# Malfoy/Brisk

Hardware: AMD Instinct MI355X
Metric: distinct k-mers indexed/sec (k=63,m=21) (higher is better)
Workload: dtype u64; 1 GPU; 1x MI355X: 50M synthetic 150 bp reads per GPU, k=63 m=21 b=14, uint8 counts, 15x coverage; reads_per_gpu=50000000, total_reads=50000000, part_bits=24, genome_len=500000000, parallelism=single GPU

## Files before the change

### brisk_amd/csrc/brisk_capi.hip

```cpp
#include "brisk_kernels.hip"

#include <algorithm>
#include <atomic>
#include <cerrno>
#include <chrono>
#include <cmath>
#include <cstdio>
#include <cstdlib>
#include <cstring>
#include <mutex>
#include <new>
#include <string>
#include <thread>
#include <vector>

#include <fcntl.h>
#include <sys/stat.h>
#include <unistd.h>

#include "../../include/brisk_hip.h"

#if !defined(__HIP_DEVICE_COMPILE__) && defined(__x86_64__)
#include <immintrin.h>
#define BRISK_HOST_AVX2 1
#endif

namespace {

enum Slot { S_PACK, S_SYNTH, S_COUNT, S_SCAN, S_HIST, S_PSUM, S_TOUCHED, S_SCATTER, S_INSERT, S_QUERY, S_ENUM, S_LOOKUP, S_PROFILE, S_PROFILE_LONG, S_UPLOAD, S_NSLOTS };
const char* const kSlotNames[S_NSLOTS] = {"k_pack_ascii", "k_synth", "k_count_kmers", "k_scan", "k_part_hist", "k_psum", "k_touched_need",
                                          "k_scatter", "k_insert", "k_query", "k_enumerate", "k_lookup", "k_profile_reads", "k_profile_segments_and_fold",
                                          "host_upload_and_pack_wall"};
static_assert(S_NSLOTS <= BRISK_HIP_PROFILE_SLOTS, "brisk_hip_profile_read fills caller arrays of BRISK_HIP_PROFILE_SLOTS");

struct DevBuf {
    void* p = nullptr;
    size_t bytes = 0;
};

struct VmBuf {
    char* base = nullptr;
    size_t reserved = 0, mapped = 0, gran = 0;
    std::vector<hipMemGenericAllocationHandle_t> handles;
    std::vector<size_t> sizes;
};

constexpr size_t kPinBytes = 8192;
struct PendingEvent {
    int slot;
    hipEvent_t a, b;
};

struct Counters {
    struct Scan { unsigned long long n_rec; u32 overflow, pad; } scan;
    struct Touched { u32 n_touched, pad; unsigned long long need; } touched;
    struct Kmers { unsigned long long bound, n_long; } kmers;
    struct Work { u32 wc[2], n_left, pad; } work;
    struct Plan { u32 n_long, n_vr; } plan;
    u32 n_rerun, pad;
    unsigned long long kept;
    unsigned long long n_ovf;
    unsigned long long slice_sum;
    u32 upsert_done, pad2;
    struct Result { unsigned long long w[3]; } result;
    unsigned long long dbg_guard;
};
static_assert(sizeof(Counters::Scan) == sizeof(unsigned long long) + 2 * sizeof(u32) && sizeof(Counters::Touched) == 2 * sizeof(u32) + sizeof(unsigned long long), "ScanOut; k_touched, k_need");
static_assert(sizeof(Counters::Kmers) == 2 * sizeof(unsigned long long) && sizeof(Counters::Result) == 3 * sizeof(unsigned long long), "k_count_kmers: out[0..1]; k_checksum: out[0..2]");
static_assert(sizeof(Counters::Work) == 4 * sizeof(u32) && sizeof(Counters::Plan) == 2 * sizeof(u32), "32-bit counters throughout");
struct PinnedCounters : Counters {
    u32 n_huge;
    unsigned long long arena_used;
    unsigned long long n_rec_new;
    unsigned long long prof[3];
    unsigned long long answers;
};

}

struct brisk_hip_index {
    BriskParams P{};
    int device = 0;
    hipStream_t stream = nullptr;
    bool own_stream = false;
    std::string err;
    std::recursive_mutex call_mu;
    u64 n_parts = 0, n_buckets = 0;
    u64 max_batch_reads = 0;

    double* d_coef = nullptr;
// ... 442 lines not shown
                           (u32)HUGE_LIST_CAP);
        if (int lrc = launch_check(h, "k_need")) return lrc;
    }
    HIPCHK(h, fetch_ctr(h, &h->d_ctr->touched.need));
    HIPCHK(h, hipMemcpyAsync(&h->h_ctr->arena_used, h->ix.cursor, 8, hipMemcpyDeviceToHost, h->stream));
    h->h_ctr->n_huge = 0;
    if (huge_at) HIPCHK(h, hipMemcpyAsync(&h->h_ctr->n_huge, h->huge.p, 4, hipMemcpyDeviceToHost, h->stream));
    HIPCHK(h, hipStreamSynchronize(h->stream));
    h->arena_used_host = h->h_ctr->arena_used;
    const u32 n_huge = h->h_ctr->n_huge <= HUGE_LIST_CAP ? h->h_ctr->n_huge : 0u;
    h->ix.huge_at = n_huge ? huge_at : 0u;
    if ((rc = ensure_arena(h, h->h_ctr->touched.need + h->h_ctr->touched.need / 7 + (u64)h->insert_waves * ARENA_CHUNK))) return rc;
    {
        ProfScope ps(h, S_INSERT);
        HIPCHK(h, zero_ctr(h, &h->d_ctr->work));
        const u32 batches = (n_touched + WI_BATCH - 1) / WI_BATCH;
        static const u64 big_at = getenv("BRISK_INSERT_BIG_AT") ? (u64)atoll(getenv("BRISK_INSERT_BIG_AT")) : 64ull;
        const bool big = !bl && n_rec / n_touched > big_at;
        const RecSrc src{bl ? bl->bins : (u64*)h->parted.p, (const u64*)h->parted.p, bl ? bl->bin_cap : 0u};
        static const u32 wave_env = getenv("BRISK_INSERT_WAVES") ? (u32)atoi(getenv("BRISK_INSERT_WAVES")) : 0u;
        const bool sat = h->count_mode == BRISK_HIP_COUNTS_SATURATE;
        auto resident = [&](const void* fn, int cap_per_cu = 0) -> u32 {
            int per_cu = 0, cus = 0;
            if (hipOccupancyMaxActiveBlocksPerMultiprocessor(&per_cu, fn, 64, 0) != hipSuccess || per_cu <= 0) per_cu = 16;
            if (cap_per_cu && per_cu > cap_per_cu) per_cu = cap_per_cu;
            if (hipDeviceGetAttribute(&cus, hipDeviceAttributeMultiprocessorCount, h->device) != hipSuccess || cus <= 0) cus = 256;
            const u32 w = std::min<u32>((u32)per_cu * (u32)cus, h->insert_waves);
            static const bool dbg = getenv("BRISK_DEBUG_INSERT") != nullptr;
            if (dbg) fprintf(stderr, "[brisk_hip] k_insert: %d waves per CU x %d CUs resident, %u launched\n", per_cu, cus, wave_env ? std::min<u32>(w, wave_env) : w);
            return wave_env ? std::min<u32>(w, wave_env) : w;
        };
        static const bool generic_only = getenv("BRISK_INSERT_GENERIC") != nullptr;
        static const bool lean_off = getenv("BRISK_INSERT_LEAN") && !strcmp(getenv("BRISK_INSERT_LEAN"), "0");
        const bool lean = fresh && !generic_only && !lean_off && !h->entry_ids && !big && P.nw == 3 && P.kb == 49 && P.shift >= 1 && P.shift <= 4;
        if (lean) {
            if ((rc = ensure(h, h->left, (size_t)n_touched * 4))) return rc;
            static const bool dbg = getenv("BRISK_DEBUG_INSERT") != nullptr;
            if (dbg) {
                hipFuncAttributes fa{};
                int per_cu = 0;
                const void* fn = sat ? (const void*)k_insert_first<3, 49, 4, true> : (const void*)k_insert_first<3, 49, 4, false>;
                if (hipFuncGetAttributes(&fa, fn) == hipSuccess && hipOccupancyMaxActiveBlocksPerMultiprocessor(&per_cu, fn, 64, 0) == hipSuccess) {
                    fprintf(stderr, "[brisk_hip] k_insert_first: the occupancy query gives %d waves per CU, the kernel is built for at most %d\n", per_cu, 4 * WI_WAVES_PER_EU_FIRST_MAX);
                    per_cu = std::min(per_cu, 4 * WI_WAVES_PER_EU_FIRST_MAX);
                    fprintf(stderr, "[brisk_hip] k_insert_first: %d waves per CU, %d registers, %zu B of LDS, %zu B of scratch\n", per_cu, fa.numRegs, fa.sharedSizeBytes, fa.localSizeBytes);
                }
            }
        }
#define LAUNCH_INSERT_K(KERNEL, NW, KB, SH, SAT)                                                                                                                    \
    {                                                                                                                                                               \
        const dim3 grid(std::min<u32>(batches, resident((const void*)KERNEL<NW, KB, SH, SAT>)));                                                                  \
        hipLaunchKernelGGL((KERNEL<NW, KB, SH, SAT>), grid, dim3(64), 0, h->stream, P, src, (const PartDesc*)h->desc.p, n_touched, h->ix,                         \
                           h->d_ctr->work.wc);                                                                                                                      \
    }
#define LAUNCH_INSERT(NW, KB, SH)                                                                                                                                   \
    {                                                                                                                                                               \
        if (big && sat) LAUNCH_INSERT_K(k_insert_big, NW, KB, SH, true)                                                                                             \
        else if (big) LAUNCH_INSERT_K(k_insert_big, NW, KB, SH, false)                                                                                              \
        else if (sat) LAUNCH_INSERT_K(k_insert, NW, KB, SH, true)                                                                                                   \
        else LAUNCH_INSERT_K(k_insert, NW, KB, SH, false)                                                                                                           \
    }
#define LAUNCH_INSERT_FAST(NW, KB, SH)                                                                                                                              \
    {                                                                                                                                                               \
        if (big) LAUNCH_INSERT(NW, KB, SH)                                                                                                                          \
        else if (sat) LAUNCH_INSERT_K(k_insert_fast, NW, KB, SH, true)                                                                                              \
        else LAUNCH_INSERT_K(k_insert_fast, NW, KB, SH, false)                                                                                                      \
    }
#define LAUNCH_INSERT_LEAN_K(SH, SAT)                                                                                                                               \
    {                                                                                                                                                               \
        u32* const wc = h->d_ctr->work.wc;                                                                                                                          \
        u32* const n_left = &h->d_ctr->work.n_left;                                                                                                                 \
        const dim3 grid(std::min<u32>(batches, resident((const void*)k_insert_first<3, 49, SH, SAT>, 4 * WI_WAVES_PER_EU_FIRST_MAX)));                                                            \
        hipLaunchKernelGGL((k_insert_first<3, 49, SH, SAT>), grid, dim3(64), 0, h->stream, P, src, (const PartDesc*)h->desc.p, n_touched, h->ix, wc,                \
                           (u32*)h->left.p, n_left);                                                                                                                \
        if ((rc = launch_check(h, "k_insert_first"))) return rc;                                                                                                    \
        const dim3 grid2(std::min<u32>(batches, resident((const void*)k_insert_fast_listed<3, 49, SH, SAT>)));                                                     \
        hipLaunchKernelGGL((k_insert_fast_listed<3, 49, SH, SAT>), grid2, dim3(64), 0, h->stream, P, src, (const PartDesc*)h->desc.p, n_touched, h->ix, wc + 1,     \
                           (const u32*)h->left.p, (const u32*)n_left);                                                                                              \
    }
#define LAUNCH_INSERT_LEAN(SH)                                                                                                                                      \
    {                                                                                                                                                               \
        if (sat) LAUNCH_INSERT_LEAN_K(SH, true)                                                                                                                     \
        else LAUNCH_INSERT_LEAN_K(SH, false)                                                                                                                        \
    }
        if (lean && P.shift == 4) LAUNCH_INSERT_LEAN(4)
        else if (lean && P.shift == 3) LAUNCH_INSERT_LEAN(3)
        else if (lean && P.shift == 2) LAUNCH_INSERT_LEAN(2)
        else if (lean) LAUNCH_INSERT_LEAN(1)
        else if (!generic_only && P.nw == 3 && P.kb == 49 && P.shift == 4) LAUNCH_INSERT_FAST(3, 49, 4)
        else if (!generic_only && P.nw == 3 && P.kb == 49 && P.shift == 3) LAUNCH_INSERT_FAST(3, 49, 3)
        else if (!generic_only && P.nw == 3 && P.kb == 49 && P.shift == 2) LAUNCH_INSERT_FAST(3, 49, 2)
        else if (!generic_only && P.nw == 3 && P.kb == 49 && P.shift == 1) LAUNCH_INSERT_FAST(3, 49, 1)
        else if (!generic_only && P.nw == 2 && P.kb == 17 && P.shift == 4) LAUNCH_INSERT_FAST(2, 17, 4)
        else if (!generic_only && P.nw == 2 && P.kb == 17 && P.shift == 5) LAUNCH_INSERT_FAST(2, 17, 5)
        else if (!generic_only && P.nw == 2 && P.kb == 17 && P.shift == 6) LAUNCH_INSERT_FAST(2, 17, 6)
        else if (!generic_only && P.nw == 2 && P.kb == 20 && P.shift == 0) LAUNCH_INSERT_FAST(2, 20, 0)
        else LAUNCH_INSERT(0, 0, 0)
#undef LAUNCH_INSERT_LEAN
#undef LAUNCH_INSERT_LEAN_K
#undef LAUNCH_INSERT_FAST
#undef LAUNCH_INSERT
#undef LAUNCH_INSERT_K
        if ((rc = launch_check(h, big ? "k_insert_big" : "k_insert"))) return rc;
        if (h->trace) {
            std::string path = big ? "k_insert_big (in-place collapse for partitions of > 128 records)" : "k_insert";
            if (lean) {
                HIPCHK(h, fetch_ctr_sync(h, &h->d_ctr->work.n_left));
                const u32 n_left = h->h_ctr->work.n_left;
                path = "k_insert_first (fresh index): " + std::to_string(n_touched - n_huge - n_left) + " partitions lean, " + std::to_string(n_left) + " left over to k_insert";
            }
            fprintf(stderr, "[brisk_hip] path: insert of %llu records (%s layout, histogram %s) into %u partitions: %s, %u partitions to k_insert_huge\n", (unsigned long long)n_rec,
                    bl ? "binned" : "classic", have_hist ? "from the scan" : "counted here", n_touched, path.c_str(), n_huge);
        }
        if (n_huge) {
            if (sat) hipLaunchKernelGGL(k_insert_huge<true>, dim3(std::min<u32>(n_huge, 256u)), dim3(HG_THREADS), 0, h->stream, P, src, (const PartDesc*)h->desc.p,
                                        (const u32*)h->huge.p + 1, (const u32*)h->huge.p, h->ix);
            else hipLaunchKernelGGL(k_insert_huge<false>, dim3(std::min<u32>(n_huge, 256u)), dim3(HG_THREADS), 0, h->stream, P, src, (const PartDesc*)h->desc.p,
                                    (const u32*)h->huge.p + 1, (const u32*)h->huge.p, h->ix);
            if ((rc = launch_check(h, "k_insert_huge"))) return rc;
        }
    }
    h->nb_skmers += n_rec;
    h->dir_snapshot_valid = false;
    return BRISK_HIP_OK;
}

int launch_scan(brisk_hip_index* h, const u32* d_packed, const u64* d_starts, u64 n_items, const ScanOut& out, bool query_mode, bool plain,
                const ChunkCtl& cc, bool pos = false) {
    ProfScope ps(h, S_SCAN);
    if (plain && !pos) {
        BriskParams P = h->P;
        if (out.ret) {
            P.ext_bits -= P.cls_bits;
            P.cls_bits = 0;
        }
        hipLaunchKernelGGL(k_scan, dim3(nblocks(n_items, SCAN_BLOCK)), dim3(SCAN_BLOCK), 0, h->stream, P, d_packed, d_starts, n_items, h->d_coef,
                           out, query_mode ? 1 : 0);
    } else {
        const u32 bt = h->scan_waves * 64;
        const dim3 grid(nblocks(n_items, bt)), block(bt);
#define LAUNCH_SCAN2(NCH, MODE, KK, MM) \
    hipLaunchKernelGGL((k_scan2<NCH, MODE, KK, MM>), grid, block, h->scan_lds - scan_fixed_tabs(MM) * 8, h->stream, h->P, h->scfg, d_packed, d_starts, n_items, h->d_tabs, out, cc)
#define LAUNCH_SCAN2_MODES(NCH, KK, MM)                    \
    {                                                      \
        if (pos && cc.vreads) LAUNCH_SCAN2(NCH, 4, KK, MM);  \
// ... 3145 lines not shown
```

### brisk_amd/csrc/brisk_insert.hip

```cpp
#ifndef ARENA_CHUNK
#define ARENA_CHUNK 16384u
#endif
#ifndef INSERT_SLOTS
#define INSERT_SLOTS 8192u
#endif
#ifndef WI_WAVES_PER_EU
#define WI_WAVES_PER_EU 4
#endif
#ifdef BRISK_PHASE_PROF
__device__ unsigned long long g_phase[16];
#define PHASE_DECL unsigned long long ph_acc[12] = {0, 0, 0, 0, 0, 0, 0, 0, 0, 0, 0, 0}; unsigned long long ph_last = __builtin_amdgcn_s_memtime(); u32 dbg_cnt[16] = {0, 0, 0, 0, 0, 0, 0, 0, 0, 0, 0, 0, 0, 0, 0, 0};
#define PHASE(i) { const unsigned long long t_ = __builtin_amdgcn_s_memtime(); ph_acc[i] += t_ - ph_last; ph_last = t_; }
__device__ unsigned long long g_cnt[16];
#define PHASE_FLUSH { PHASE(10) if (threadIdx.x == 0) { _Pragma("unroll") for (int q_ = 0; q_ < 12; q_++) atomicAdd(&g_phase[q_], ph_acc[q_]); \
                                                         _Pragma("unroll") for (int q_ = 0; q_ < 16; q_++) atomicAdd(&g_cnt[q_], (unsigned long long)dbg_cnt[q_]); } }
#define CNT(i, v) dbg_cnt[i] += (v);
#else
#define PHASE_DECL
#define PHASE(i)
#define PHASE_FLUSH
#define CNT(i, v)
#endif
struct IndexDev {
    u64* keys;
// ... 196 lines not shown
                    hh[it] = (hh[it] + 1) & (tsize - 1);
                }
            }
        }
    }
}

template <u32 NW>
struct RecGeom {
    static constexpr u32 CW = 2 * NW + 1;
    static constexpr u32 RS = 2 * NW + 3;
    static constexpr u32 INFO = 2 * NW + 1;
};
template <u32 NW>
__device__ __forceinline__ void store_rec_words(u32* dst, const RecRegs& rr, u32 info) {
    const u64 c0 = rr.w0, c1 = NW > 1 ? rr.w1 : 0, c2 = NW > 2 ? rr.w2 : 0, c3 = NW > 3 ? rr.w3 : 0;
    const u64 s0 = c0 << 6, s1 = (c1 << 6) | (c0 >> 58), s2 = (c2 << 6) | (c1 >> 58), s3 = (c3 << 6) | (c2 >> 58);
    const u32 top = (u32)((NW == 1 ? c0 : NW == 2 ? c1 : NW == 3 ? c2 : c3) >> 58);
    dst[0] = (u32)s0;
    dst[1] = (u32)(s0 >> 32);
    if (NW > 1) { dst[2] = (u32)s1; dst[3] = (u32)(s1 >> 32); }
    if (NW > 2) { dst[4] = (u32)s2; dst[5] = (u32)(s2 >> 32); }
    if (NW > 3) { dst[6] = (u32)s3; dst[7] = (u32)(s3 >> 32); }
    dst[2 * NW] = top;
    dst[RecGeom<NW>::INFO] = info;
    dst[RecGeom<NW>::INFO + 1] = 0;
}
template <u32 NIMAX>
struct LaneInst {
    u64 klo[NIMAX], khi[NIMAX];
    u32 hh[NIMAX];
    u32 won;
};
template <u32 NI, u32 NW, u32 KB, u32 SHIFT, u32 NIMAX, bool FOLD, bool SAT>
__device__ __forceinline__ void expand_and_dedupe_words(u32 lane, u32 ninst, u32 tsize, const u32* s_rw, const uint8_t* s_irec, const uint8_t* s_imult,
                                                        const u32* s_rmult, u64* s_key, u32* s_tab, u32* dbg_rounds, LaneInst<NIMAX>& li) {
    constexpr u32 RS = RecGeom<NW>::RS, INFO = RecGeom<NW>::INFO, KBITS = 2 * KB + 6;
    static_assert(KBITS + SHIFT <= 128 && SHIFT <= 6, "entry key: [routing id low bits | compacted k-mer | idx']");
    static_assert(NI <= NIMAX, "instances per lane");
    u64 (&klo)[NIMAX] = li.klo;
    u64 (&khi)[NIMAX] = li.khi;
    u32 (&hh)[NIMAX] = li.hh;
    u32 mult[NI];
    u32 rix[NI];
    u32 won = 0;
#pragma unroll
    for (u32 it = 0; it < NI; it++) {
        const u32 i = it * 64 + lane;
        rix[it] = s_irec[i < ninst ? i : 0];
    }
#pragma unroll
    for (u32 it = 0; it < NI; it++) {
        const u32 i = it * 64 + lane;
        const u32* base = s_rw + rix[it] * RS;
        const u32 info = base[INFO];
        const u32 j = i < ninst ? i - (info & 0x3ffu) : 0;
        const u32 n = (info >> 10) & 0xffu;
        const u32 s = 2 * (n - 1 - j);
        const u32* wp = base + (s >> 5);
        const u32 sh = s & 31;
        const u32 w0 = wp[0], w1 = wp[1], w2 = wp[2], w3 = wp[3], w4 = wp[4];
        u32 k0 = __builtin_amdgcn_alignbit(w1, w0, sh), k1 = __builtin_amdgcn_alignbit(w2, w1, sh);
        u32 k2 = __builtin_amdgcn_alignbit(w3, w2, sh), k3 = __builtin_amdgcn_alignbit(w4, w3, sh);
        k0 = (k0 & ~0x3fu) | (((info >> 18) & 0xffu) + j);
        constexpr u32 m0 = KBITS >= 32 ? ~0u : (1u << KBITS) - 1, m1 = KBITS >= 64 ? ~0u : KBITS <= 32 ? 0u : (1u << (KBITS - 32)) - 1;
        constexpr u32 m2 = KBITS >= 96 ? ~0u : KBITS <= 64 ? 0u : (1u << (KBITS - 64)) - 1, m3 = KBITS >= 128 ? ~0u : KBITS <= 96 ? 0u : (1u << (KBITS - 96)) - 1;
        k0 &= m0; k1 &= m1; k2 &= m2; k3 &= m3;
        u64 lo = ((u64)k1 << 32) | k0, hi = ((u64)k3 << 32) | k2;
        if (SHIFT) {
            const u64 rl = (info >> 26) & ((1u << SHIFT) - 1);
            if (KBITS >= 64) hi |= rl << (KBITS - 64);
            else {
                lo |= rl << KBITS;
                if (KBITS + SHIFT > 64) hi |= rl >> (64 - KBITS);
            }
        }
        klo[it] = lo;
        khi[it] = hi;
        hh[it] = hash_key32(mk128(lo, hi)) & (tsize - 1);
        mult[it] = FOLD ? (u32)s_imult[i < ninst ? i : 0] << WI_CNT_SHIFT : count8<SAT>(s_rmult[rix[it]]) << WI_CNT_SHIFT;
        if (i < ninst) {
            s_key[2 * i] = lo;
            s_key[2 * i + 1] = hi;
        }
    }
    wave_sync();
    for (u32 w = 0; w * 64 < tsize; w++) s_tab[w * 64 + lane] = EMPTY_SLOT;
    wave_sync();
    u32 pending = 0;
#pragma unroll
    for (u32 it = 0; it < NI; it++)
        if (it * 64 + lane < ninst) pending |= 1u << it;
    while (__any(pending != 0)) {
        *dbg_rounds += NI;
        u32 old[NI];
#pragma unroll
        for (u32 it = 0; it < NI; it++) {
            old[it] = EMPTY_SLOT;
            if (pending >> it & 1) old[it] = atomicCAS(&s_tab[hh[it]], EMPTY_SLOT, (it * 64 + lane) | mult[it]);
        }
        u64 olo[NI], ohi[NI];
#pragma unroll
        for (u32 it = 0; it < NI; it++) {
            const u32 oi = old[it] == EMPTY_SLOT ? 0 : (old[it] & WI_IDX_MASK);
            olo[it] = s_key[2 * oi];
            ohi[it] = s_key[2 * oi + 1];
        }
#pragma unroll
        for (u32 it = 0; it < NI; it++) {
// ... 41 lines not shown
                break;
            }
            h = (h + 1) & (2 * WI_MAX_REC - 1);
        }
    }
    return dup;
}

#ifndef WI_FOLD_TRIPS
#define WI_FOLD_TRIPS 16u
#endif
struct FoldFrame {
    W4 u, m;
    u32 rid;
    u32 rng;
    u32 s;
};
template <u32 NW, u32 KB>
__device__ __forceinline__ FoldFrame fold_frame(const RecRegs& rr, u64 hdr, u32 n, bool valid, u32 frame_end, u32 lane) {
    FoldFrame f;
    const u32 idx0 = hdr_idx0(hdr), end = idx0 + n, top = frame_end - idx0 + KB - 1;
    const bool ok = valid && n > 0 && end <= frame_end && top <= 32 * NW;
    const u32 lo_bits = ok ? 2 * (frame_end - end) : 0, hi_bits = ok ? 2 * top : 0;
    f.m = w4_andn(w4_mask(hi_bits), w4_mask(lo_bits));
    f.u = w4_and(w4_shl(W4{rr.w0, NW > 1 ? rr.w1 : 0, NW > 2 ? rr.w2 : 0, NW > 3 ? rr.w3 : 0}, lo_bits), f.m);
    f.rid = hdr_bucket(hdr);
    f.rng = idx0 | (end << 8);
    f.s = ok ? (n << 6) | (63 - lane) : 0;
    return f;
}
__device__ __forceinline__ u64 readlane64(u64 v, u32 a) {
    return ((u64)(u32)__builtin_amdgcn_readlane((int)(v >> 32), (int)a) << 32) | (u32)__builtin_amdgcn_readlane((int)v, (int)a);
}
template <u32 NW>
__device__ __forceinline__ bool fold_records(const FoldFrame& f, u32 nrec, u32 lane, u32* lead, u32* off, u32* trips) {
    u32 sv = lane < nrec ? f.s : 0;
    bool folded = false;
    *lead = lane;
    *off = 0;
    for (u32 t = 0; t < WI_FOLD_TRIPS; t++) {
        const u32 smax = (u32)__builtin_amdgcn_readlane((int)wave_incl_max_scan(sv), 63);
        if (smax == 0) break;
        *trips += 1;
        const u32 a = 63 - (smax & 63);
        const u32 rid_a = (u32)__builtin_amdgcn_readlane((int)f.rid, (int)a), rng_a = (u32)__builtin_amdgcn_readlane((int)f.rng, (int)a);
        const u32 i0 = f.rng & 0xffu, e = f.rng >> 8, i0a = rng_a & 0xffu, ea = rng_a >> 8;
#ifdef BRISK_NO_RECORD_FOLD
        bool in = sv != 0 && rid_a == f.rid && i0a == i0 && ea == e;
#else
        bool in = sv != 0 && rid_a == f.rid && i0a <= i0 && e <= ea;
#endif
        bool same = (readlane64(f.u.w0, a) & f.m.w0) == f.u.w0;
        if (NW > 1) same = same & ((readlane64(f.u.w1, a) & f.m.w1) == f.u.w1);
        if (NW > 2) same = same & ((readlane64(f.u.w2, a) & f.m.w2) == f.u.w2);
        if (NW > 3) same = same & ((readlane64(f.u.w3, a) & f.m.w3) == f.u.w3);
        in = in && same;
        if (in) {
            sv = 0;
            if (lane != a) {
                folded = true;
                *lead = a;
                *off = i0 - i0a;
            }
        }
    }
    return folded;
}

template <u32 MAXI, u32 NW, u32 KB, u32 SHIFT, bool SAT, bool LISTED = false>
__device__ __forceinline__ void insert_body(const BriskParams& PP, const RecSrc& src, const PartDesc* __restrict__ desc, u32 n_touched_all, const IndexDev& ix,
                                            u32* __restrict__ work_counter, const u32* __restrict__ list = nullptr, const u32* __restrict__ n_list = nullptr) {
    const u32 n_touched = LISTED ? min(*n_list, n_touched_all) : n_touched_all;
    u64* const rec = src.rec;
    BriskParams P = PP;
    if (NW) {
        P.nw = NW;
        P.stride = NW + 1;
        P.kb = KB;
        P.shift = SHIFT;
    }
    constexpr u32 TABLE = 2 * MAXI, TS = TABLE / 64, NI = MAXI / 64;
    constexpr u32 KW = NW ? (2 * KB + 6 + SHIFT <= 64 ? 1u : 2u) : 0u;
    constexpr bool FOLD = NW >= 3 && MAXI == WI_MAX_INST;
    static_assert(MAXI % 256 == 0 && MAXI <= 1024, "chunk size: whole 32-bit words of record marks per lane, 10-bit instance index");
    constexpr u32 REC_U64 = WI_MAX_REC * 5 > MAXI / 2 ? WI_MAX_REC * 5 : MAXI / 2;
    static_assert(NW == 0 || (WI_MAX_REC * RecGeom<NW ? NW : 1>::RS + 4) * 4 <= REC_U64 * 8, "shifted record words must fit the record buffer");
    constexpr bool TAB_OVER_REC = NW && TABLE * 4 <= REC_U64 * 8;
    constexpr u32 OFF_REC = 16 * MAXI, OFF_TAB = TAB_OVER_REC ? OFF_REC : OFF_REC + 8 * REC_U64, OFF_RTAB = TAB_OVER_REC ? OFF_REC + 8 * REC_U64 : OFF_TAB + 4 * TABLE;
    constexpr u32 OFF_RMULT = OFF_RTAB + 4 * 2 * WI_MAX_REC, OFF_IREC = OFF_RMULT + 4 * WI_MAX_REC, OFF_PREF = OFF_IREC + MAXI;
    constexpr u32 LDS_BYTES = NW ? OFF_PREF : OFF_PREF + 4 * (WI_MAX_REC + 1) + 4;
    __shared__ __attribute__((aligned(16))) unsigned char s_mem[LDS_BYTES];
    u64* s_key = (u64*)s_mem;
    u32* s_idiff = (u32*)s_mem;
    u64* s_rec = (u64*)(s_mem + OFF_REC);
    u32* s_rw = (u32*)s_rec;
    u32* s_tab = (u32*)(s_mem + OFF_TAB);
    u32* s_list = (u32*)s_rec;
    u32* s_rtab = (u32*)(s_mem + OFF_RTAB);
// ... 392 lines not shown
__global__ void __launch_bounds__(64) __attribute__((amdgpu_waves_per_eu(WI_WAVES_PER_EU, 8))) k_insert(BriskParams P, RecSrc src, const PartDesc* __restrict__ desc,
                                               u32 n_touched, IndexDev ix, u32* __restrict__ work_counter) {
    insert_body<WI_MAX_INST, NW, KB, SHIFT, SAT>(P, src, desc, n_touched, ix, work_counter);
}
template <u32 NW, u32 KB, u32 SHIFT, bool SAT = false>
__global__ void __launch_bounds__(64) __attribute__((amdgpu_waves_per_eu(2, 8))) k_insert_big(BriskParams P, RecSrc src, const PartDesc* __restrict__ desc,
                                                                                         u32 n_touched, IndexDev ix, u32* __restrict__ work_counter) {
    insert_body<2 * WI_MAX_INST, NW, KB, SHIFT, SAT>(P, src, desc, n_touched, ix, work_counter);
}

#ifndef NI_LEAN
#define NI_LEAN 3
#endif
#ifndef WI_WAVES_PER_EU_FIRST
#define WI_WAVES_PER_EU_FIRST 6
#endif
#ifndef WI_WAVES_PER_EU_FIRST_MAX
#define WI_WAVES_PER_EU_FIRST_MAX 6
#endif
template <u32 NIL, u32 NW>
struct LeanLds {
    static constexpr u32 MAXI = 64 * NIL, TABLE = 512;
    static_assert((TABLE & (TABLE - 1)) == 0 && TABLE >= 2 * MAXI && TABLE <= 4 * MAXI, "probe table: a power of two, at most half full");
    static constexpr u32 REC_BYTES = (WI_MAX_REC * RecGeom<NW>::RS + 4) * 4;
    static constexpr u32 OFF_REC = 16 * MAXI;
    static constexpr u32 REGION = REC_BYTES > 4 * TABLE ? REC_BYTES : 4 * TABLE;
    static constexpr u32 OFF_IREC = OFF_REC + REGION, OFF_IMULT = OFF_IREC + MAXI, BYTES = OFF_IMULT + MAXI;
};
__device__ __forceinline__ unsigned long long first_lane64(unsigned long long v) {
    return ((unsigned long long)(u32)__builtin_amdgcn_readfirstlane((int)(v >> 32)) << 32) | (u32)__builtin_amdgcn_readfirstlane((int)v);
}
template <u32 NIL, u32 NW, u32 KB, u32 SHIFT, bool SAT>
__device__ __forceinline__ void insert_first_body(const BriskParams& P, const RecSrc& src, const PartDesc* __restrict__ desc, u32 n_touched, const IndexDev& ix,
                                                  u32* __restrict__ work_counter, u32* __restrict__ left_list, u32* __restrict__ n_left) {
    using L = LeanLds<NIL, NW>;
    constexpr u32 MAXI = L::MAXI, TABLE = L::TABLE, RS = RecGeom<NW>::RS, INFO = RecGeom<NW>::INFO, KBITS = 2 * KB + 6;
    constexpr u32 KW = KBITS + SHIFT <= 64 ? 1u : 2u;
    static_assert(NIL == 2 || NIL == 3, "instance slots per lane");
    static_assert(NW >= 3 && SHIFT < 5, "the folding k63 geometries: at most 16 buckets per partition");
    static_assert(L::BYTES <= 13 * 512, "LDS per wave: 24 waves must fit a CU's 160 KiB");
    static_assert(4 * MAXI <= 16 * MAXI, "the multiplicity steps lie over the keys");
    static_assert(MAXI + (MAXI >> 2) + 8 <= ARENA_CHUNK / 8, "grow_cap(MAXI) is a small request: the host's arena reserve covers the tail a refill strands");
    __shared__ __attribute__((aligned(16))) unsigned char s_mem[L::BYTES];
    u64* s_key = (u64*)s_mem;
    u32* s_idiff = (u32*)s_mem;
    u32* s_rw = (u32*)(s_mem + L::OFF_REC);
    u32* s_tab = (u32*)(s_mem + L::OFF_REC);
    uint8_t* s_irec = s_mem + L::OFF_IREC;
    uint8_t* s_imult = s_mem + L::OFF_IMULT;

    const u32 lane = threadIdx.x;
    PHASE_DECL
    unsigned long long acur = first_lane64(ix.slot_cur[blockIdx.x]), aend = first_lane64(ix.slot_end[blockIdx.x]), garbage = 0;
    const u32 frame_end = P.suff_reduc + P.w + 1;

    for (;;) {
        u32 t0 = 0;
        if (lane == 0) t0 = atomicAdd(work_counter, WI_BATCH);
        t0 = (u32)__builtin_amdgcn_readfirstlane((int)t0);
        if (t0 >= n_touched) break;
        const u32 t_end = min(t0 + WI_BATCH, n_touched);
        unsigned long long left_mask = 0;
        PartDesc d = desc[t0];
        RecRegs rr = load_part_recs(P, src, d.part, d.r_begin, d.r_begin, min(d.n_rec, (u32)WI_MAX_REC), lane);

        for (u32 t = t0; t < t_end; t++) {
            const u32 tn = t + 1;
            PartDesc dn{};
            if (tn < t_end) dn = desc[tn];
            asm volatile("" ::"v"(rr.w0), "v"(rr.w1), "v"(rr.w2), "v"(rr.w3), "v"(rr.w4));
            do {
                if (ix.huge_at && d.n_inst > ix.huge_at) break;
                CNT(0, 1)
                if (d.n_exist | d.cap | (u32)(d.n_rec > WI_MAX_REC)) {
                    left_mask |= 1ull << (t - t0);
                    break;
                }
                PHASE(0)
                const u32 part = d.part, nrec = d.n_rec;
                const u64 my_hdr = NW == 3 ? rr.w3 : rr.w4;
                const u32 raw_n = lane < nrec ? hdr_n(my_hdr) : 0;
                const u32 my_mult = (my_hdr & HDR_HAS_MULT) ? (u32)(my_hdr >> 48) & 0xffu : 1u;
                const u32 info_hi = (raw_n << 10) | (hdr_idx0(my_hdr) << 18) | ((hdr_bucket(my_hdr) & ((1u << SHIFT) - 1)) << 26);
                const FoldFrame ff = fold_frame<NW, KB>(rr, my_hdr, raw_n, lane < nrec, frame_end, lane);
                wave_sync();
                if (lane < nrec) store_rec_words<NW>(s_rw + lane * RS, rr, 0);
                u32 lead = lane, lead_off = 0, dbg_trips = 0;
                const bool dup = fold_records<NW>(ff, nrec, lane, &lead, &lead_off, &dbg_trips);
                const u32 my_n = (lane < nrec && !dup) ? raw_n : 0;
                const u32 x = wave_incl_scan(my_n, lane);
                const u32 ninst = (u32)__builtin_amdgcn_readlane((int)x, 63);
                if (ninst > MAXI) {
                    left_mask |= 1ull << (t - t0);
                    break;
                }
                PHASE(1)
                CNT(1, 1)
                const u32 m_first = (u32)__shfl(x - my_n, lead, 64) + lead_off;
                u32 tsize = 128;
                while (tsize < 4 * ninst && tsize < TABLE) tsize <<= 1;
                {
                    if (NIL == 2) ((uint16_t*)s_irec)[lane] = 0;
                    else {
#pragma unroll
                        for (u32 q = 0; q < NIL; q++) s_irec[q * 64 + lane] = 0;
                    }
#pragma unroll
                    for (u32 q = 0; q < NIL; q++) s_idiff[lane * NIL + q] = 0;
                    wave_sync();
                    if (my_n) s_irec[x - my_n] = (uint8_t)(lane + 1);
                    if (lane < nrec) {
                        atomicAdd(&s_idiff[m_first], my_mult);
                        if (m_first + raw_n < ninst) atomicAdd(&s_idiff[m_first + raw_n], 0u - my_mult);
                    }
                    wave_sync();
                    u32 mk[NIL], mv[NIL], run = 0, tot = 0;
                    if (NIL == 2) {
                        const u32 w = ((const uint16_t*)s_irec)[lane];
                        mk[0] = w & 0xff;
                        mk[1] = w >> 8;
                    } else {
// ... 5 lines not shown
                        run = op_max_u32(run, mk[q]);
                        tot += s_idiff[lane * NIL + q];
                        mv[q] = tot;
                    }
                    const u32 before = wave_incl_scan(tot, lane) - tot;
                    u32 carry = wave_prev_lane(wave_incl_max_scan(run));
#pragma unroll
                    for (u32 q = 0; q < NIL; q++) {
                        carry = op_max_u32(carry, mk[q]);
                        mk[q] = (carry - 1) & 0xff;
                        mv[q] = count8<SAT>(mv[q] + before) & 0xff;
                    }
                    if (NIL == 2) {
                        ((uint16_t*)s_irec)[lane] = (uint16_t)(mk[0] | (mk[1] << 8));
                        ((uint16_t*)s_imult)[lane] = (uint16_t)(mv[0] | (mv[1] << 8));
                    } else {
#pragma unroll
                        for (u32 q = 0; q < NIL; q++) {
                            s_irec[lane * NIL + q] = (uint8_t)mk[q];
                            s_imult[lane * NIL + q] = (uint8_t)mv[q];
                        }
                    }
                    if (lane < nrec) s_rw[lane * RS + INFO] = (x - my_n) | info_hi;
                }
                wave_sync();
                PHASE(2)
                CNT(3, (ninst + 63) / 64)
                CNT(4, ninst)
                CNT(5, nrec)
                CNT(11, dbg_trips)
                u32 dbg_r = 0;
                LaneInst<NIL> li;
                li.won = 0;
                if (ninst <= 64) expand_and_dedupe_words<1, NW, KB, SHIFT, NIL, true, SAT>(lane, ninst, tsize, s_rw, s_irec, s_imult, nullptr, s_key, s_tab, &dbg_r, li);
                else if (NIL == 2 || ninst <= 128) expand_and_dedupe_words<2, NW, KB, SHIFT, NIL, true, SAT>(lane, ninst, tsize, s_rw, s_irec, s_imult, nullptr, s_key, s_tab, &dbg_r, li);
                else expand_and_dedupe_words<NIL, NW, KB, SHIFT, NIL, true, SAT>(lane, ninst, tsize, s_rw, s_irec, s_imult, nullptr, s_key, s_tab, &dbg_r, li);
                wave_sync();
                CNT(8, dbg_r)
                PHASE(3)
                u32 n_new = 0, new_rank[NIL], new_word[NIL];
#pragma unroll
                for (u32 it = 0; it < NIL; it++) {
                    new_rank[it] = 0;
                    new_word[it] = 0;
                    if (it * 64 < ninst) {
                        const bool made = (li.won >> it) & 1;
                        if (made) new_word[it] = s_tab[li.hh[it]];
                        const unsigned long long bal = __ballot(made);
                        new_rank[it] = n_new + (u32)__popcll(bal & lanes_below(lane));
                        n_new += (u32)__popcll(bal);
                    }
                }
                wave_sync();
#ifndef INSERT_NO_EARLY_WAIT
                __builtin_amdgcn_s_waitcnt(0x0F70);
#endif
                PHASE(6)
                CNT(7, n_new)
                unsigned long long off = d.off;
                u32 cap = 0;
                if (n_new) {
                    const unsigned long long want = grow_cap(n_new);
                    if (acur + want > aend) {
                        garbage += aend - acur;
                        unsigned long long got = 0;
                        if (lane == 0) got = atomicAdd(ix.cursor, (unsigned long long)ARENA_CHUNK);
                        acur = first_lane64(got);
                        aend = acur + ARENA_CHUNK;
                    }
                    if (acur + want > ix.arena_cap) {
                        if (lane == 0) atomicOr(ix.err, 2u);
                        n_new = 0;
                    } else {
                        off = acur;
                        acur += want;
                        cap = (u32)want;
                    }
                }
                PHASE(7)
                u32 bm0 = 0;
#pragma unroll
                for (u32 it = 0; it < NIL; it++) {
                    if (it * 64 < ninst && ((li.won >> it) & 1) && n_new) {
                        const unsigned long long at = off + new_rank[it];
                        store_key<KW>(ix, at, li.klo[it], li.khi[it]);
                        ix.counts[at] = (uint8_t)count8<SAT>(new_word[it] >> WI_CNT_SHIFT);
                        const u32 bl = SHIFT ? ((u32)shr128(mk128(li.klo[it], li.khi[it]), KBITS).lo & ((1u << SHIFT) - 1)) : 0;
                        bm0 |= 1u << bl;
                    }
                }
                PHASE(8)
                bm0 = wave_or_all(bm0);
                if (lane == 0) {
                    ix.dir[part] = DirEnt{off, n_new, cap};
                    const u64 first = ((u64)part << SHIFT) >> P.ext_bits;
                    const u32 bits = bm0 << (first & 31);
                    if (bits && (!ix.bits_check || (ix.bucket_bits[first >> 5] & bits) != bits)) atomicOr(&ix.bucket_bits[first >> 5], bits);
                }
            } while (0);
            d = dn;
            if (tn < t_end) rr = load_part_recs(P, src, d.part, d.r_begin, d.r_begin, min(d.n_rec, (u32)WI_MAX_REC), lane);
            PHASE(9)
        }
        if (left_mask) {
            const u32 n = (u32)__popcll(left_mask);
            u32 at = 0;
            if (lane == 0) at = atomicAdd(n_left, n);
            at = (u32)__builtin_amdgcn_readfirstlane((int)at);
            if ((left_mask >> lane) & 1) left_list[at + (u32)__popcll(left_mask & lanes_below(lane))] = t0 + lane;
        }
    }
    PHASE_FLUSH
    if (lane == 0) {
        ix.slot_cur[blockIdx.x] = acur;
        ix.slot_end[blockIdx.x] = aend;
        if (garbage) atomicAdd(&ix.stats[3], garbage);
    }
}
template <u32 NW, u32 KB, u32 SHIFT, bool SAT = false, u32 NIL = NI_LEAN>
__global__ void __launch_bounds__(64) __attribute__((amdgpu_waves_per_eu(WI_WAVES_PER_EU_FIRST, WI_WAVES_PER_EU_FIRST_MAX))) k_insert_first(BriskParams P, RecSrc src, const PartDesc* __restrict__ desc,
                                                                                                          u32 n_touched, IndexDev ix, u32* __restrict__ work_counter,
                                                                                                          u32* __restrict__ left_list, u32* __restrict__ n_left) {
    insert_first_body<NIL, NW, KB, SHIFT, SAT>(P, src, desc, n_touched, ix, work_counter, left_list, n_left);
}

__global__ void __launch_bounds__(256) k_bucket_bits(BriskParams P, IndexDev ix, u32 n_parts) {
    const u32 kbits = 2 * P.kb + 6;
    for (u32 part = blockIdx.x; part < n_parts; part += gridDim.x) {
        const u32 cnt = ix.dir[part].cnt;
        const unsigned long long off = ix.dir[part].off;
        for (u32 e = threadIdx.x; e < cnt; e += blockDim.x) {
            const u128x key = load_key(ix, off + e);
            const u32 bucket = (part << P.shift) | ((u32)shr128(key, kbits).lo & ((1u << P.shift) - 1));
            const u32 bit = 1u << (bucket & 31);
            if (!(ix.bucket_bits[bucket >> 5] & bit)) atomicOr(&ix.bucket_bits[bucket >> 5], bit);
        }
    }
}

__global__ void __launch_bounds__(256) k_stats(const DirEnt* __restrict__ dir, u64 n_parts, const u32* __restrict__ bits, u64 n_words,
                                               unsigned long long* out ) {
    __shared__ unsigned long long s_a[4], s_b[4], s_c[4];
    unsigned long long a = 0, b = 0, c = 0;
    const u64 stride = (u64)gridDim.x * blockDim.x;
    for (u64 i = (u64)blockIdx.x * blockDim.x + threadIdx.x; i < n_parts; i += stride) {
        const u32 v = dir[i].cnt;
        a += v;
        c = v > c ? v : c;
    }
    for (u64 i = (u64)blockIdx.x * blockDim.x + threadIdx.x; i < n_words; i += stride) b += __popc(bits[i]);
    for (int o = 32; o > 0; o >>= 1) {
        a += __shfl_down(a, o, 64);
        b += __shfl_down(b, o, 64);
        const unsigned long long c2 = __shfl_down(c, o, 64);
        c = c2 > c ? c2 : c;
    }
// ... 211 lines not shown
```

Measured before the change: 29.61 billion k-mers/s.

## Skip LDS hash-table dedupe in lean insert when fold proves instances distinct

During record folding, the fresh-index lean insert path now checks whether any two records that share a minimizer core could produce overlapping k-mer instances. When none can, the partition is marked clean and its keys are expanded directly without the LDS hash-table dedupe, and ranks are assigned by instance index. This removes the hashing, table probing and extra wave syncs for most partitions. In exchange it adds a readlane comparison per fold trip, more register pressure in the hot kernel, a counter atomic, and a correctness risk if the distinctness test misses a duplicate.

```diff
diff --git a/brisk_amd/csrc/brisk_capi.hip b/brisk_amd/csrc/brisk_capi.hip
--- a/brisk_amd/csrc/brisk_capi.hip
+++ b/brisk_amd/csrc/brisk_capi.hip
@@ -55,7 +55,7 @@
     struct Scan { unsigned long long n_rec; u32 overflow, pad; } scan;
     struct Touched { u32 n_touched, pad; unsigned long long need; } touched;
     struct Kmers { unsigned long long bound, n_long; } kmers;
-    struct Work { u32 wc[2], n_left, pad; } work;
+    struct Work { u32 wc[2], n_left, n_clean; } work;
     struct Plan { u32 n_long, n_vr; } plan;
     u32 n_rerun, pad;
     unsigned long long kept;
@@ -564,6 +564,7 @@
         };
         static const bool generic_only = getenv("BRISK_INSERT_GENERIC") != nullptr;
         static const bool lean_off = getenv("BRISK_INSERT_LEAN") && !strcmp(getenv("BRISK_INSERT_LEAN"), "0");
+        static const bool clean_off = getenv("BRISK_INSERT_CLEAN") && !strcmp(getenv("BRISK_INSERT_CLEAN"), "0");
         const bool lean = fresh && !generic_only && !lean_off && !h->entry_ids && !big && P.nw == 3 && P.kb == 49 && P.shift >= 1 && P.shift <= 4;
         if (lean) {
             if ((rc = ensure(h, h->left, (size_t)n_touched * 4))) return rc;
@@ -602,9 +603,10 @@
     {                                                                                                                                                               \
         u32* const wc = h->d_ctr->work.wc;                                                                                                                          \
         u32* const n_left = &h->d_ctr->work.n_left;                                                                                                                 \
+        u32* const n_clean = clean_off ? nullptr : &h->d_ctr->work.n_clean;                                                                                         \
         const dim3 grid(std::min<u32>(batches, resident((const void*)k_insert_first<3, 49, SH, SAT>, 4 * WI_WAVES_PER_EU_FIRST_MAX)));                                                            \
         hipLaunchKernelGGL((k_insert_first<3, 49, SH, SAT>), grid, dim3(64), 0, h->stream, P, src, (const PartDesc*)h->desc.p, n_touched, h->ix, wc,                \
-                           (u32*)h->left.p, n_left);                                                                                                                \
+                           (u32*)h->left.p, n_left, n_clean);                                                                                                       \
         if ((rc = launch_check(h, "k_insert_first"))) return rc;                                                                                                    \
         const dim3 grid2(std::min<u32>(batches, resident((const void*)k_insert_fast_listed<3, 49, SH, SAT>)));                                                     \
         hipLaunchKernelGGL((k_insert_fast_listed<3, 49, SH, SAT>), grid2, dim3(64), 0, h->stream, P, src, (const PartDesc*)h->desc.p, n_touched, h->ix, wc + 1,     \
@@ -635,14 +637,15 @@
 #undef LAUNCH_INSERT_K
         if ((rc = launch_check(h, big ? "k_insert_big" : "k_insert"))) return rc;
         if (h->trace) {
-            std::string path = big ? "k_insert_big (in-place collapse for partitions of > 128 records)" : "k_insert";
+            std::string path = big ? "k_insert_big (in-place collapse for partitions of > 128 records)" : "k_insert", tail;
             if (lean) {
-                HIPCHK(h, fetch_ctr_sync(h, &h->d_ctr->work.n_left));
+                HIPCHK(h, fetch_ctr_sync(h, &h->d_ctr->work));
                 const u32 n_left = h->h_ctr->work.n_left;
                 path = "k_insert_first (fresh index): " + std::to_string(n_touched - n_huge - n_left) + " partitions lean, " + std::to_string(n_left) + " left over to k_insert";
+                tail = " (" + std::to_string(h->h_ctr->work.n_clean) + " table-free)";
             }
-            fprintf(stderr, "[brisk_hip] path: insert of %llu records (%s layout, histogram %s) into %u partitions: %s, %u partitions to k_insert_huge\n", (unsigned long long)n_rec,
-                    bl ? "binned" : "classic", have_hist ? "from the scan" : "counted here", n_touched, path.c_str(), n_huge);
+            fprintf(stderr, "[brisk_hip] path: insert of %llu records (%s layout, histogram %s) into %u partitions: %s, %u partitions to k_insert_huge%s\n", (unsigned long long)n_rec,
+                    bl ? "binned" : "classic", have_hist ? "from the scan" : "counted here", n_touched, path.c_str(), n_huge, tail.c_str());
         }
         if (n_huge) {
             if (sat) hipLaunchKernelGGL(k_insert_huge<true>, dim3(std::min<u32>(n_huge, 256u)), dim3(HG_THREADS), 0, h->stream, P, src, (const PartDesc*)h->desc.p,
diff --git a/brisk_amd/csrc/brisk_insert.hip b/brisk_amd/csrc/brisk_insert.hip
--- a/brisk_amd/csrc/brisk_insert.hip
+++ b/brisk_amd/csrc/brisk_insert.hip
@@ -252,10 +252,56 @@
     u32 hh[NIMAX];
     u32 won;
 };
+template <u32 NW, u32 KB, u32 SHIFT>
+__device__ __forceinline__ void cut_key(const u32* base, u32 i, u32 ninst, u64* lo_out, u64* hi_out) {
+    constexpr u32 INFO = RecGeom<NW>::INFO, KBITS = 2 * KB + 6;
+    const u32 info = base[INFO];
+    const u32 j = i < ninst ? i - (info & 0x3ffu) : 0;
+    const u32 n = (info >> 10) & 0xffu;
+    const u32 s = 2 * (n - 1 - j);
+    const u32* wp = base + (s >> 5);
+    const u32 sh = s & 31;
+    const u32 w0 = wp[0], w1 = wp[1], w2 = wp[2], w3 = wp[3], w4 = wp[4];
+    u32 k0 = __builtin_amdgcn_alignbit(w1, w0, sh), k1 = __builtin_amdgcn_alignbit(w2, w1, sh);
+    u32 k2 = __builtin_amdgcn_alignbit(w3, w2, sh), k3 = __builtin_amdgcn_alignbit(w4, w3, sh);
+    k0 = (k0 & ~0x3fu) | (((info >> 18) & 0xffu) + j);
+    constexpr u32 m0 = KBITS >= 32 ? ~0u : (1u << KBITS) - 1, m1 = KBITS >= 64 ? ~0u : KBITS <= 32 ? 0u : (1u << (KBITS - 32)) - 1;
+    constexpr u32 m2 = KBITS >= 96 ? ~0u : KBITS <= 64 ? 0u : (1u << (KBITS - 64)) - 1, m3 = KBITS >= 128 ? ~0u : KBITS <= 96 ? 0u : (1u << (KBITS - 96)) - 1;
+    k0 &= m0; k1 &= m1; k2 &= m2; k3 &= m3;
+    u64 lo = ((u64)k1 << 32) | k0, hi = ((u64)k3 << 32) | k2;
+    if (SHIFT) {
+        const u64 rl = (info >> 26) & ((1u << SHIFT) - 1);
+        if (KBITS >= 64) hi |= rl << (KBITS - 64);
+        else {
+            lo |= rl << KBITS;
+            if (KBITS + SHIFT > 64) hi |= rl >> (64 - KBITS);
+        }
+    }
+    *lo_out = lo;
+    *hi_out = hi;
+}
+template <u32 NI, u32 NW, u32 KB, u32 SHIFT, u32 NIMAX>
+__device__ __forceinline__ void expand_words_distinct(u32 lane, u32 ninst, const u32* s_rw, const uint8_t* s_irec, LaneInst<NIMAX>& li) {
+    static_assert(NI <= NIMAX, "instances per lane");
+    u32 rix[NI];
+    u32 won = 0;
+#pragma unroll
+    for (u32 it = 0; it < NI; it++) {
+        const u32 i = it * 64 + lane;
+        rix[it] = s_irec[i < ninst ? i : 0];
+    }
+#pragma unroll
+    for (u32 it = 0; it < NI; it++) {
+        const u32 i = it * 64 + lane;
+        cut_key<NW, KB, SHIFT>(s_rw + rix[it] * RecGeom<NW>::RS, i, ninst, &li.klo[it], &li.khi[it]);
+        if (i < ninst) won |= 1u << it;
+    }
+    li.won = won;
+}
 template <u32 NI, u32 NW, u32 KB, u32 SHIFT, u32 NIMAX, bool FOLD, bool SAT>
 __device__ __forceinline__ void expand_and_dedupe_words(u32 lane, u32 ninst, u32 tsize, const u32* s_rw, const uint8_t* s_irec, const uint8_t* s_imult,
                                                         const u32* s_rmult, u64* s_key, u32* s_tab, u32* dbg_rounds, LaneInst<NIMAX>& li) {
-    constexpr u32 RS = RecGeom<NW>::RS, INFO = RecGeom<NW>::INFO, KBITS = 2 * KB + 6;
+    constexpr u32 RS = RecGeom<NW>::RS, KBITS = 2 * KB + 6;
     static_assert(KBITS + SHIFT <= 128 && SHIFT <= 6, "entry key: [routing id low bits | compacted k-mer | idx']");
     static_assert(NI <= NIMAX, "instances per lane");
     u64 (&klo)[NIMAX] = li.klo;
@@ -272,29 +318,8 @@
 #pragma unroll
     for (u32 it = 0; it < NI; it++) {
         const u32 i = it * 64 + lane;
-        const u32* base = s_rw + rix[it] * RS;
-        const u32 info = base[INFO];
-        const u32 j = i < ninst ? i - (info & 0x3ffu) : 0;
-        const u32 n = (info >> 10) & 0xffu;
-        const u32 s = 2 * (n - 1 - j);
-        const u32* wp = base + (s >> 5);
-        const u32 sh = s & 31;
-        const u32 w0 = wp[0], w1 = wp[1], w2 = wp[2], w3 = wp[3], w4 = wp[4];
-        u32 k0 = __builtin_amdgcn_alignbit(w1, w0, sh), k1 = __builtin_amdgcn_alignbit(w2, w1, sh);
-        u32 k2 = __builtin_amdgcn_alignbit(w3, w2, sh), k3 = __builtin_amdgcn_alignbit(w4, w3, sh);
-        k0 = (k0 & ~0x3fu) | (((info >> 18) & 0xffu) + j);
-        constexpr u32 m0 = KBITS >= 32 ? ~0u : (1u << KBITS) - 1, m1 = KBITS >= 64 ? ~0u : KBITS <= 32 ? 0u : (1u << (KBITS - 32)) - 1;
-        constexpr u32 m2 = KBITS >= 96 ? ~0u : KBITS <= 64 ? 0u : (1u << (KBITS - 64)) - 1, m3 = KBITS >= 128 ? ~0u : KBITS <= 96 ? 0u : (1u << (KBITS - 96)) - 1;
-        k0 &= m0; k1 &= m1; k2 &= m2; k3 &= m3;
-        u64 lo = ((u64)k1 << 32) | k0, hi = ((u64)k3 << 32) | k2;
-        if (SHIFT) {
-            const u64 rl = (info >> 26) & ((1u << SHIFT) - 1);
-            if (KBITS >= 64) hi |= rl << (KBITS - 64);
-            else {
-                lo |= rl << KBITS;
-                if (KBITS + SHIFT > 64) hi |= rl >> (64 - KBITS);
-            }
-        }
+        u64 lo, hi;
+        cut_key<NW, KB, SHIFT>(s_rw + rix[it] * RS, i, ninst, &lo, &hi);
         klo[it] = lo;
         khi[it] = hi;
         hh[it] = hash_key32(mk128(lo, hi)) & (tsize - 1);
@@ -402,10 +427,20 @@
 __device__ __forceinline__ u64 readlane64(u64 v, u32 a) {
     return ((u64)(u32)__builtin_amdgcn_readlane((int)(v >> 32), (int)a) << 32) | (u32)__builtin_amdgcn_readlane((int)v, (int)a);
 }
-template <u32 NW>
-__device__ __forceinline__ bool fold_records(const FoldFrame& f, u32 nrec, u32 lane, u32* lead, u32* off, u32* trips) {
+template <u32 KB, u32 CW>
+__device__ __forceinline__ u32 fold_core(const W4& u) {
+    constexpr u32 LO = 2 * CW, N = 2 * (KB - CW), WI = LO / 64, BI = LO % 64;
+    static_assert(CW < KB && N <= 28 && LO + N <= 256, "the core: the minimizer's nucleotides that are not cut out, m - b of them");
+    const u64 w[5] = {u.w0, u.w1, u.w2, u.w3, 0};
+    u64 v = w[WI] >> BI;
+    if (BI + N > 64) v |= w[WI + 1] << (64 - BI);
+    return (u32)v & ((1u << N) - 1);
+}
+template <u32 NW, bool DETECT = false>
+__device__ __forceinline__ bool fold_records(const FoldFrame& f, u32 nrec, u32 lane, u32* lead, u32* off, u32* trips, u32 ck = 0, bool unsure = false, bool* clean = nullptr) {
     u32 sv = lane < nrec ? f.s : 0;
     bool folded = false;
+    u32 dirty = unsure;
     *lead = lane;
     *off = 0;
     for (u32 t = 0; t < WI_FOLD_TRIPS; t++) {
@@ -433,7 +468,13 @@
                 *off = i0 - i0a;
             }
         }
-    }
+        if (DETECT) {
+            const u32 differs = ck ^ (u32)__builtin_amdgcn_readlane((int)ck, (int)a);
+            const u32 meets = ((i0 - ea) & (i0a - e)) >> 31;
+            dirty |= (differs == 0 && sv != 0) ? meets : 0u;
+        }
+    }
+    if (DETECT) *clean = !__any((dirty | sv) != 0);
     return folded;
 }
 
@@ -892,10 +933,12 @@
 }
 template <u32 NIL, u32 NW, u32 KB, u32 SHIFT, bool SAT>
 __device__ __forceinline__ void insert_first_body(const BriskParams& P, const RecSrc& src, const PartDesc* __restrict__ desc, u32 n_touched, const IndexDev& ix,
-                                                  u32* __restrict__ work_counter, u32* __restrict__ left_list, u32* __restrict__ n_left) {
+                                                  u32* __restrict__ work_counter, u32* __restrict__ left_list, u32* __restrict__ n_left, u32* __restrict__ n_clean) {
     using L = LeanLds<NIL, NW>;
     constexpr u32 MAXI = L::MAXI, TABLE = L::TABLE, RS = RecGeom<NW>::RS, INFO = RecGeom<NW>::INFO, KBITS = 2 * KB + 6;
     constexpr u32 KW = KBITS + SHIFT <= 64 ? 1u : 2u;
+    constexpr u32 CORE_K = 63, CORE_M = 21, CORE_B = 14, CW = CORE_K - CORE_M;
+    static_assert(KB == CORE_K - CORE_B, "fold_core: the core of k63 m21 b14");
     static_assert(NIL == 2 || NIL == 3, "instance slots per lane");
     static_assert(NW >= 3 && SHIFT < 5, "the folding k63 geometries: at most 16 buckets per partition");
     static_assert(L::BYTES <= 13 * 512, "LDS per wave: 24 waves must fit a CU's 160 KiB");
@@ -913,6 +956,7 @@
     PHASE_DECL
     unsigned long long acur = first_lane64(ix.slot_cur[blockIdx.x]), aend = first_lane64(ix.slot_end[blockIdx.x]), garbage = 0;
     const u32 frame_end = P.suff_reduc + P.w + 1;
+    const u32 core_from = (n_clean != nullptr && P.w == CW) ? P.suff_reduc : 0x100u;
 
     for (;;) {
         u32 t0 = 0;
@@ -921,6 +965,7 @@
         if (t0 >= n_touched) break;
         const u32 t_end = min(t0 + WI_BATCH, n_touched);
         unsigned long long left_mask = 0;
+        unsigned long long clean_mask = 0;
         PartDesc d = desc[t0];
         RecRegs rr = load_part_recs(P, src, d.part, d.r_begin, d.r_begin, min(d.n_rec, (u32)WI_MAX_REC), lane);
 
@@ -946,7 +991,13 @@
                 wave_sync();
                 if (lane < nrec) store_rec_words<NW>(s_rw + lane * RS, rr, 0);
                 u32 lead = lane, lead_off = 0, dbg_trips = 0;
-                const bool dup = fold_records<NW>(ff, nrec, lane, &lead, &lead_off, &dbg_trips);
+                const bool unsure = lane < nrec && (ff.s == 0 || hdr_idx0(my_hdr) < core_from);
+                bool clean = false;
+                const u32 ck = ((hdr_bucket(my_hdr) & ((1u << SHIFT) - 1)) << (2 * (KB - CW))) | fold_core<KB, CW>(ff.u);
+                const bool dup = fold_records<NW, true>(ff, nrec, lane, &lead, &lead_off, &dbg_trips, ck, unsure, &clean);
+#ifdef INSERT_ATTR_NOTABLE
+                clean = true;
+#endif
                 const u32 my_n = (lane < nrec && !dup) ? raw_n : 0;
                 const u32 x = wave_incl_scan(my_n, lane);
                 const u32 ninst = (u32)__builtin_amdgcn_readlane((int)x, 63);
@@ -1018,23 +1069,40 @@
                 u32 dbg_r = 0;
                 LaneInst<NIL> li;
                 li.won = 0;
-                if (ninst <= 64) expand_and_dedupe_words<1, NW, KB, SHIFT, NIL, true, SAT>(lane, ninst, tsize, s_rw, s_irec, s_imult, nullptr, s_key, s_tab, &dbg_r, li);
-                else if (NIL == 2 || ninst <= 128) expand_and_dedupe_words<2, NW, KB, SHIFT, NIL, true, SAT>(lane, ninst, tsize, s_rw, s_irec, s_imult, nullptr, s_key, s_tab, &dbg_r, li);
-                else expand_and_dedupe_words<NIL, NW, KB, SHIFT, NIL, true, SAT>(lane, ninst, tsize, s_rw, s_irec, s_imult, nullptr, s_key, s_tab, &dbg_r, li);
-                wave_sync();
-                CNT(8, dbg_r)
-                PHASE(3)
                 u32 n_new = 0, new_rank[NIL], new_word[NIL];
-#pragma unroll
-                for (u32 it = 0; it < NIL; it++) {
-                    new_rank[it] = 0;
-                    new_word[it] = 0;
-                    if (it * 64 < ninst) {
-                        const bool made = (li.won >> it) & 1;
-                        if (made) new_word[it] = s_tab[li.hh[it]];
-                        const unsigned long long bal = __ballot(made);
-                        new_rank[it] = n_new + (u32)__popcll(bal & lanes_below(lane));
-                        n_new += (u32)__popcll(bal);
+                if (clean) {
+                    clean_mask |= 1ull << (t - t0);
+                    u32 ln = lane;
+                    asm volatile("" : "+v"(ln));
+                    if (ninst <= 64) expand_words_distinct<1, NW, KB, SHIFT, NIL>(ln, ninst, s_rw, s_irec, li);
+                    else if (NIL == 2 || ninst <= 128) expand_words_distinct<2, NW, KB, SHIFT, NIL>(ln, ninst, s_rw, s_irec, li);
+                    else expand_words_distinct<NIL, NW, KB, SHIFT, NIL>(ln, ninst, s_rw, s_irec, li);
+                    n_new = ninst;
+#pragma unroll
+                    for (u32 it = 0; it < NIL; it++) {
+                        const u32 i = it * 64 + ln;
+                        new_rank[it] = i;
+                        new_word[it] = (u32)s_imult[i < ninst ? i : 0] << WI_CNT_SHIFT;
+                    }
+                    PHASE(3)
+                } else {
+                    if (ninst <= 64) expand_and_dedupe_words<1, NW, KB, SHIFT, NIL, true, SAT>(lane, ninst, tsize, s_rw, s_irec, s_imult, nullptr, s_key, s_tab, &dbg_r, li);
+                    else if (NIL == 2 || ninst <= 128) expand_and_dedupe_words<2, NW, KB, SHIFT, NIL, true, SAT>(lane, ninst, tsize, s_rw, s_irec, s_imult, nullptr, s_key, s_tab, &dbg_r, li);
+                    else expand_and_dedupe_words<NIL, NW, KB, SHIFT, NIL, true, SAT>(lane, ninst, tsize, s_rw, s_irec, s_imult, nullptr, s_key, s_tab, &dbg_r, li);
+                    wave_sync();
+                    CNT(8, dbg_r)
+                    PHASE(3)
+#pragma unroll
+                    for (u32 it = 0; it < NIL; it++) {
+                        new_rank[it] = 0;
+                        new_word[it] = 0;
+                        if (it * 64 < ninst) {
+                            const bool made = (li.won >> it) & 1;
+                            if (made) new_word[it] = s_tab[li.hh[it]];
+                            const unsigned long long bal = __ballot(made);
+                            new_rank[it] = n_new + (u32)__popcll(bal & lanes_below(lane));
+                            n_new += (u32)__popcll(bal);
+                        }
                     }
                 }
                 wave_sync();
@@ -1093,8 +1161,11 @@
             u32 at = 0;
             if (lane == 0) at = atomicAdd(n_left, n);
             at = (u32)__builtin_amdgcn_readfirstlane((int)at);
-            if ((left_mask >> lane) & 1) left_list[at + (u32)__popcll(left_mask & lanes_below(lane))] = t0 + lane;
-        }
+            u32 ln = lane;
+            asm volatile("" : "+v"(ln));
+            if ((left_mask >> ln) & 1) left_list[at + (u32)__popcll(left_mask & lanes_below(ln))] = t0 + ln;
+        }
+        if (clean_mask && n_clean && lane == 0) atomicAdd(n_clean, (u32)__popcll(clean_mask));
     }
     PHASE_FLUSH
     if (lane == 0) {
@@ -1106,8 +1177,8 @@
 template <u32 NW, u32 KB, u32 SHIFT, bool SAT = false, u32 NIL = NI_LEAN>
 __global__ void __launch_bounds__(64) __attribute__((amdgpu_waves_per_eu(WI_WAVES_PER_EU_FIRST, WI_WAVES_PER_EU_FIRST_MAX))) k_insert_first(BriskParams P, RecSrc src, const PartDesc* __restrict__ desc,
                                                                                                           u32 n_touched, IndexDev ix, u32* __restrict__ work_counter,
-                                                                                                          u32* __restrict__ left_list, u32* __restrict__ n_left) {
-    insert_first_body<NIL, NW, KB, SHIFT, SAT>(P, src, desc, n_touched, ix, work_counter, left_list, n_left);
+                                                                                                          u32* __restrict__ left_list, u32* __restrict__ n_left, u32* __restrict__ n_clean) {
+    insert_first_body<NIL, NW, KB, SHIFT, SAT>(P, src, desc, n_touched, ix, work_counter, left_list, n_left, n_clean);
 }
 
 __global__ void __launch_bounds__(256) k_bucket_bits(BriskParams P, IndexDev ix, u32 n_parts) {
```

New measurement: 30.80 billion k-mers/s (median of 6 runs). 1.04x the previous value.
